# mehrnazmo/VIforSSMs

Hardware: AMD Instinct MI355X
Metric: latent-state transitions/sec (batch_dims×T per step), AR(1) T=5000, 1/2/4/8 GPU (higher is better)
Workload: dtype bf16

## Files before the change

viforssms_amd/csrc/flow_v5.hip:

```cpp
#include "flow5_api.hpp"

#ifndef VISSM_FLOW5_NS
#define VISSM_FLOW5_NS flow5
#define VISSM_FLOW5_BASE_UNIT 1
#endif

#include <cstdlib>
#ifndef VISSM_ABL_STORES
#define VISSM_ABL_STORES 0
#endif

namespace vissm {
namespace VISSM_FLOW5_NS {

constexpr int P = 16;
constexpr int HP = 64;
constexpr int S = 16;
constexpr int NW = 4;
constexpr int NT = 64 * NW;
constexpr int UW = 128;
constexpr int DTH = 56;

typedef __bf16 bf4 __attribute__((ext_vector_type(4)));
typedef __bf16 bf8 __attribute__((ext_vector_type(8)));
// ... 949 lines not shown
                for (int j = 0; j + w2 < KF; j += 2 * w2) t[j] += t[j + w2];
              v = t[0];
            } else {
#pragma unroll 4
              for (int j = 0; j < a.k; ++j) v += dsc[j * QW + qc];
            }
          } else {
#pragma unroll
            for (int p = 0; p < P; ++p) {
              const int j = q - a.s * p;
              const bool ok = static_cast<unsigned>(j) < static_cast<unsigned>(a.k);
              const float x = dsc[(ok ? j : 0) * QW + p];
              v += ok ? x : 0.f;
            }
          }
          const int oq2 = q - a.k;
          if (oq2 >= 0 && oq2 < fin) {
            if (a.s == 1) v += gw[oq2] * gsc[w][0][oq2];
            else v += (oq2 & 1) ? gw[oq2] * gsc[w][0][oq2 >> 1] : gsc[w][2][oq2 >> 1];
          }
          const float cin = mycarry[bl * KP + (q < a.k ? q : 0)];
          if (q < a.k) v += cin;
          if (q < fin) db[t0 + q] = v;
          else if (q < fin + a.k) mycarry[bl * KP + q - fin] = v;
        }
      }
    }
    if (c < nP) {
      const size_t row = (static_cast<size_t>(grp) * a.Lh + m0 + c) * a.H;
      if (a.dc16) {
        __bf16* dcs = reinterpret_cast<__bf16*>(dC_slab) + row;
#pragma unroll
        for (int rb = 0; rb < 4; ++rb)
#pragma unroll
          for (int r = 0; r < 4; ++r) {
            const int h = swz(16 * rb + 4 * g + r);
            if (h < a.H) dcs[h] = static_cast<__bf16>(dCa[rb][r] * kLog2e);
          }
      } else {
        float* dcs = dC_slab + row;
#pragma unroll
        for (int rb = 0; rb < 4; ++rb)
#pragma unroll
          for (int r = 0; r < 4; ++r) {
            const int h = swz(16 * rb + 4 * g + r);
            if (h < a.H) dcs[h] = dCa[rb][r] * kLog2e;
          }
      }
    }
  }

  if constexpr (FZ) {
    if (lane < nb) {
      float v = 0.f;
#pragma unroll
      for (int cc = 0; cc < P; ++cc) v += zls[w][lane][cc];
      fz.lsl[static_cast<size_t>(chn) * a.B + b_lo + lane] = v;
    }
  }
  for (int bl = 0; bl < nb; ++bl) {
    const int b = b_lo + bl;
    for (int q = lane; q < a.k * wdu; q += 64) {
      const float v = mycarry[bl * KP + q];
      if (chn == a.n_chunks - 1) du[static_cast<size_t>(b) * a.pL + a.Lout + q] = v;
      else halo[(static_cast<size_t>(b) * a.n_chunks + chn) * a.k + q] = v;
    }
    if (lane < a.H) dth_slab[(static_cast<size_t>(chn) * a.B + b) * a.H + lane] = dthl[w][bl][swz(lane)] * kLog2e;
  }

  const int H = a.H;
  const int nW = a.k * H + NH * H * H + 3 * NH * H + 2 * H + 2;
  float* ws = dW_slab + static_cast<size_t>(item) * nW;
#pragma unroll
  for (int jb = 0; jb < JB; ++jb)
#pragma unroll
    for (int hb = 0; hb < 4; ++hb)
#pragma unroll
      for (int r = 0; r < 4; ++r) {
        const int j = 16 * jb + 4 * g + r, h = swz(16 * hb + c);
        if (j < a.k && h < H) ws[j * H + h] = dWe[jb][hb][r] * kLog2e;
      }
  const int off_w = a.k * H, off_b = off_w + NH * H * H;
#pragma unroll
  for (int l = 0; l < NH; ++l)
#pragma unroll
    for (int ib = 0; ib < 4; ++ib)
#pragma unroll
      for (int ob = 0; ob < 4; ++ob)
#pragma unroll
        for (int r = 0; r < 4; ++r) {
          const int hi = swz(16 * ib + 4 * g + r), ho = swz(16 * ob + c);
          if (ho < H) {
            if (hi < H) ws[off_w + (l * H + hi) * H + ho] = dW[l][ib][ob][r];
            else if (hi == 63) ws[off_b + l * H + ho] = dW[l][ib][ob][r] * kLog2e;
          }
        }
  for (int i = lane; i < 2 * NH * H; i += 64) ws[off_b + NH * H + i] = 0.f;
  const int off_h = off_b + 3 * NH * H;
  const int oh = GI ? c - 5 : c;
  if (oh == 0 || oh == 1) {
#pragma unroll
    for (int hb = 0; hb < 4; ++hb)
#pragma unroll
      for (int r = 0; r < 4; ++r) {
        const int h = swz(16 * hb + 4 * g + r);
        if (h < H) ws[off_h + h * 2 + oh] = dWh[hb][r] * kLn2;
        else if (h == 63) ws[off_h + 2 * H + oh] = dWh[hb][r];
      }
  }
}

constexpr int NW2 = 8;
constexpr int NT2 = 64 * NW2;
__device__ __forceinline__ float swap_hi_lo(float v) {
  const auto r = __builtin_amdgcn_permlane32_swap(__builtin_bit_cast(unsigned, v), __builtin_bit_cast(unsigned, v),
                                                  false, false);
  return __builtin_bit_cast(float, static_cast<unsigned>(r[1]));
}
constexpr int KP2 = 8;
#ifndef VISSM_NODU_FENCES
#define VISSM_NODU_FENCES 1
#endif
template <bool FZ>
__device__ __forceinline__ void fence2() {
  if constexpr (FZ) fence();
}
#ifndef VISSM_BWD2_AHEAD
#define VISSM_BWD2_AHEAD 2
#endif
#ifndef VISSM_BWD2_AHEAD_VAR
#define VISSM_BWD2_AHEAD_VAR 6
#endif
#ifndef VISSM_BWD2_TAIL_DU
#define VISSM_BWD2_TAIL_DU 5
#endif
#ifndef VISSM_BWD2_TAIL_FZ
#define VISSM_BWD2_TAIL_FZ 59
#endif
#ifndef VISSM_BWD2_TAIL_NODU
#define VISSM_BWD2_TAIL_NODU 4
#endif
#ifndef VISSM_STAGE_AHEAD
#define VISSM_STAGE_AHEAD 1
#endif
#ifndef VISSM_STAGE_AHEAD_VAR
#define VISSM_STAGE_AHEAD_VAR 12
#endif
#ifndef VISSM_STAGE_SITE_DU
#define VISSM_STAGE_SITE_DU 0
#endif
#ifndef VISSM_STAGE_SITE_FZ
#define VISSM_STAGE_SITE_FZ 2
#endif
__device__ __forceinline__ unsigned lds_addr(const void* p) {
  return __builtin_amdgcn_readfirstlane(
      static_cast<unsigned>(reinterpret_cast<size_t>((__attribute__((address_space(3))) const void*)p)));
}
__device__ __forceinline__ void lds_dma_pair(unsigned long long mask0, unsigned long long mask1, unsigned voff,
                                             const float* base0, const float* base1, unsigned dst0, unsigned dst1) {
  unsigned keep_m0;
  unsigned long long keep_exec;
  asm volatile(
      "s_nop 4\n\t"
      "s_mov_b32 %0, m0\n\t"
      "s_and_saveexec_b64 %1, %2\n\t"
      "s_mov_b32 m0, %7\n\t"
      "s_nop 0\n\t"
      "global_load_lds_dword %4, %5\n\t"
      "s_and_b64 exec, %1, %3\n\t"
      "s_mov_b32 m0, %8\n\t"
      "s_nop 0\n\t"
      "global_load_lds_dword %4, %6\n\t"
      "s_mov_b64 exec, %1\n\t"
      "s_mov_b32 m0, %0"
      : "=&s"(keep_m0), "=&s"(keep_exec)
      : "s"(mask0), "s"(mask1), "v"(voff), "s"(base0), "s"(base1), "s"(dst0), "s"(dst1)
      : "memory", "scc");
}
__device__ __forceinline__ unsigned long long lanes_below(int n, bool on) {
  return on ? (n >= 64 ? ~0ull : (1ull << n) - 1ull) : 0ull;
}
template <int N>
__device__ __forceinline__ void stage_windows(const float* src, int pitch, int len, int b0, int b1, int t0, int n,
                                              int lane, float (*win)[N], bool on, bool both) {
  const unsigned long long m = lanes_below(n, on);
  lds_dma_pair(m, both ? m : 0ull, 4u * static_cast<unsigned>(clampi(t0 + lane, len)),
               src + static_cast<size_t>(b0) * pitch, src + static_cast<size_t>(b1) * pitch, lds_addr(win[0]),
               lds_addr(win[1]));
}
__device__ __forceinline__ void stage_wait() { asm volatile("s_waitcnt vmcnt(0)" ::: "memory"); }

constexpr int kSgMfma = 0x008, kSgDsRead = 0x100;
template <int ID, int N, int M>
__device__ __forceinline__ void sg_batch() {
  __builtin_amdgcn_sched_group_barrier(kSgDsRead, N, ID);
#pragma unroll
  for (int i = 0; i < N; ++i) __builtin_amdgcn_sched_group_barrier(kSgMfma, M, ID);
}
template <int ID, int NR, int NM>
__device__ __forceinline__ void sg_seq() {
  __builtin_amdgcn_sched_group_barrier(kSgDsRead, NR, ID);
  __builtin_amdgcn_sched_group_barrier(kSgMfma, NM, ID);
}

__device__ __forceinline__ bf8 cat8(bf4 a, bf4 b) {
  return __builtin_shufflevector(a, b, 0, 1, 2, 3, 4, 5, 6, 7);
}
__device__ __forceinline__ bf8 tr_frag2(const __bf16* img, int hb, int g, int c) {
  return cat8(tr_read(img, hb, g, c), tr_read(img + P * HP, hb, g, c));
}

#define VISSM_UW (*(STG ? &uwin[pw + w] : &uwin[w]))
#define VISSM_GW (*(STGG ? &gwin[pw + w] : &gwin[w]))
template <bool FZ, bool DU, bool TF, int NPR = 1, bool SB = false>
__global__ __launch_bounds__(NT2, 2) void bwd2_kernel(KArgs a, const float* __restrict__ u, const float* __restrict__ C,
                                                      const float* __restrict__ tht, const float* __restrict__ gout,
                                                      const float* __restrict__ dls, const bf8* __restrict__ img,
                                                      const float* __restrict__ cst, float* __restrict__ du,
                                                      float* __restrict__ dC_slab, float* __restrict__ dth_slab,
                                                      float* __restrict__ dW_slab, float* __restrict__ halo,
                                                      const u4* __restrict__ thf, FzArgs fz = FzArgs{}) {
  static_assert(!SB || NPR == 2, "the split backward chain goes with the split recompute");
  constexpr int NH = 1, KB = 1, JB = 1, NP = 1;
  constexpr bool LOF = NPR == 2 && !kLoFoldOff;
  constexpr bool AH =
      VISSM_BWD2_AHEAD && NPR == 1 && (FZ || TF) && (VISSM_BWD2_AHEAD_VAR & (FZ ? 4 : DU ? 2 : 1)) != 0;
  constexpr int TAIL = (VISSM_BWD2_AHEAD >= 2 && NPR == 1 && TF)
                           ? (FZ ? VISSM_BWD2_TAIL_FZ : DU ? VISSM_BWD2_TAIL_DU : VISSM_BWD2_TAIL_NODU) : 0;
  constexpr int PO = FZ ? P - 1 : P;
  constexpr int QW2 = P + KP2;
  constexpr int UWN = NPR == 2 ? 48 : 64;
  __shared__ Shared<NH, KB, JB, NP> sh;
  __shared__ __bf16 timg[NW2][2][2 * P * HP];
  __shared__ float dthl[NW2][S][DTH];
  __shared__ __attribute__((aligned(16))) float dths[NW2][4];
  __shared__ float carry[NW2][S][KP2];
  constexpr bool STG = VISSM_STAGE_AHEAD && NPR == 1 && TF && UWN == 64 &&
                       (VISSM_STAGE_AHEAD_VAR & (FZ ? 8 : DU ? 4 : 2)) != 0;
  constexpr bool STGG = STG && !FZ;
  constexpr int SITE = FZ ? VISSM_STAGE_SITE_FZ : VISSM_STAGE_SITE_DU;
  __shared__ float uwin[STG ? 2 * NW2 : NW2][2][UWN];
  __shared__ float gwin[STGG ? 2 * NW2 : NW2][2][P];
  __shared__ float gsc[NPR == 2 ? 1 : NW2][2][P];
  __shared__ float dscr[NW2][2][KP2][QW2];
  constexpr bool ZLS = FZ && NPR == 1;
  __shared__ float zls[ZLS ? NW2 : 1][ZLS ? S : 1][P];
  constexpr int RO = NPR == 2 ? 10 : 0, NLO = RO + (SB ? 10 : 0);
  __shared__ bf8 slo[NLO > 0 ? NLO : 1][64];
  __shared__ bf8 swe[NPR == 2 ? 4 : 1][16];
  __shared__ float zcar[FZ ? NW2 : 1][FZ ? S : 1];
  if constexpr (NPR == 2) {
    constexpr int NFR = Shared<NH, KB, JB, NP>::NFR;
    for (int i = threadIdx.x; i < NFR * 64; i += NT2) sh.img[i >> 6][0][i & 63] = img[((i >> 6) * 2) * 64 + (i & 63)];
    for (int i = threadIdx.x; i < NLO * 64; i += NT2) {
      const int j = i >> 6;
      const int f = j < 8 ? j
                  : j < 10 ? 16 * NH + 4 * KB + 2 * JB + (j - 8)
                  : j < 18 ? 8 * NH + (j - 10)
                           : 16 * NH + 4 * KB + (j - 18);
      slo[j][i & 63] = img[(f * 2 + 1) * 64 + (i & 63)];
    }
    for (int i = threadIdx.x; i < 4 * 16; i += NT2) swe[i >> 4][i & 15] = img[((16 * NH + (i >> 4)) * 2 + 1) * 64 + (i & 15)];
    for (int i = threadIdx.x; i < Shared<NH, KB, JB, NP>::NCST; i += NT2) sh.cst[i] = cst[i];
  } else {
    load_shared<NH, KB, JB, NP, NT2>(sh, img, cst);
  }
  if constexpr (FZ) {
    if constexpr (ZLS)
      for (int i = threadIdx.x; i < NW2 * S * P; i += NT2) (&zls[0][0][0])[i] = 0.f;
    for (int i = threadIdx.x; i < NW2 * S; i += NT2) (&zcar[0][0])[i] = 0.f;
  }
  for (int i = threadIdx.x; i < NW2 * S * DTH; i += NT2) (&dthl[0][0][0])[i] = 0.f;
  for (int i = threadIdx.x; i < NW2 * S * KP2; i += NT2) (&carry[0][0][0])[i] = 0.f;
  for (int i = threadIdx.x; i < NW2 * 2 * KP2 * QW2; i += NT2) (&dscr[0][0][0][0])[i] = 0.f;
  __syncthreads();
  const int w = threadIdx.x >> 6, lane = threadIdx.x & 63, c = lane & 15, g = lane >> 4;
  const int item = __builtin_amdgcn_readfirstlane(blockIdx.x * NW2 + w);
  const int grp = __builtin_amdgcn_readfirstlane(item / a.n_chunks);
  const int chn = __builtin_amdgcn_readfirstlane(item % a.n_chunks);
  if (grp >= a.n_groups) return;
  const int m_lo = chn * a.CH, m_hi = min(a.Lh, m_lo + a.CH);
  const int b_lo = grp * a.S, nb = min(a.S, a.B - b_lo);
  __bf16* const im0 = timg[w][0];
  __bf16* const im1 = timg[w][1];
  const unsigned* whp = reinterpret_cast<const unsigned*>(&sh.cst[NH * HP]);

  f4 dW[4][4], dWe[4], dWh[4];
#pragma unroll
  for (int i = 0; i < 4; ++i) {
#pragma unroll
    for (int o = 0; o < 4; ++o) dW[i][o] = f4{0.f, 0.f, 0.f, 0.f};
    dWe[i] = f4{0.f, 0.f, 0.f, 0.f};
    dWh[i] = f4{0.f, 0.f, 0.f, 0.f};
  }
  const int fwc = 16 * NH + 4 * KB;
  bf8 sel_p;
#pragma unroll
  for (int jj = 0; jj < 8; ++jj) sel_p[jj] = (__bf16)((4 * g + (jj & 3) == c) ? 1.f : 0.f);

  const float ldl = (!FZ && lane < nb) ? dls[b_lo + lane] : 0.f;
  float lt0 = 0.f, lt1 = 0.f, lis = 0.f;
  if constexpr (FZ) {
    if (lane < nb) {
      const float* tp = fz.theta + static_cast<size_t>(b_lo + lane) * 3;
      lt0 = tp[0];
      lt1 = tp[1];
      lis = __expf(-tp[2]);
    }
  }
  const int m_start = (FZ && chn > 0) ? m_lo - PO : m_lo;
  const int nu = a.k + P;
  int par = 0;
  if constexpr (STG) {
    if (lane >= nu) {
#pragma unroll
      for (int cb = 0; cb < 2; ++cb) {
        uwin[w][cb][lane] = 0.f;
        uwin[NW2 + w][cb][lane] = 0.f;
      }
    }
    stage_windows(u, a.pL, a.L, b_lo, b_lo + (1 < nb ? 1 : 0), m_start, nu, lane, uwin[w], m_start < m_hi, true);
    if constexpr (!FZ)
      stage_windows(gout, a.pLo, a.Lout, b_lo, b_lo + (1 < nb ? 1 : 0), m_start, P, lane, gwin[w], m_start < m_hi,
                    1 < nb);
  }
  for (int m0 = m_start; m0 < m_hi; m0 += PO) {
    const bool discard = FZ && m0 < m_lo;
    const int nP = discard ? 0 : min(PO, m_hi - m0), t0 = m0;
    const int nZ = FZ ? min(P, a.Lh - m0) : nP;
    f4 dCa[4];
#pragma unroll
    for (int rb = 0; rb < 4; ++rb) dCa[rb] = f4{0.f, 0.f, 0.f, 0.f};
    float fz_yt = 0.f, fz_bt = 0.f;
    if constexpr (FZ) {
      const int wo = min(max(m0 + c - 1, 0), fz.M - 1);
      fz_yt = fz.obs[wo];
      fz_bt = fz.bin[wo];
    }
    for (int bl = 0; bl < nb; bl += 2) {
      fence2<FZ || (!DU && VISSM_NODU_FENCES)>();
      const bool two = bl + 1 < nb;
      const int blv[2] = {bl, two ? bl + 1 : bl};
      const int bv[2] = {b_lo + blv[0], b_lo + blv[1]};
      int pw = 0;
      if constexpr (STG) {
        stage_wait();
        pw = par * NW2;
        asm volatile("" : "+s"(pw));
      }
      const auto stage_next = [&]() {
        const bool lastp = bl + 2 >= nb, more = !lastp || m0 + PO < m_hi;
        const int ms = (lastp && more) ? m0 + PO : m0, bs = lastp ? (more ? 0 : bl) : bl + 2;
        const int b0 = b_lo + bs, b1 = b_lo + (bs + 1 < nb ? bs + 1 : bs);
        __builtin_amdgcn_sched_barrier(0);
        stage_windows(u, a.pL, a.L, b0, b1, ms, nu, lane, uwin[NW2 - pw + w], more, true);
        if constexpr (STGG)
          stage_windows(gout, a.pLo, a.Lout, b0, b1, ms, P, lane, gwin[NW2 - pw + w], more, bs + 1 < nb);
        __builtin_amdgcn_sched_barrier(0);
      };
      (void)stage_next;
      f4 X[2][4];
      bf8 tfr[2];
      float fz_yp = fz_yt, fz_bp = fz_bt, fz_zc[2] = {0.f, 0.f};
      {
        float uv[2] = {0.f, 0.f}, gv[2] = {0.f, 0.f};
        if constexpr (!STG) {
#pragma unroll
          for (int cb = 0; cb < 2; ++cb) {
            const float* ub = u + static_cast<size_t>(bv[cb]) * a.pL;
            uv[cb] = lane < nu ? ub[clampi(t0 + lane, a.L)] : 0.f;
            if constexpr (!FZ) {
              if (lane < P) gv[cb] = gout[static_cast<size_t>(bv[cb]) * a.pLo + clampi(t0 + lane, a.Lout)];
            }
          }
          if (!two) gv[1] = 0.f;
        }
        const f4* crow = reinterpret_cast<const f4*>(C + static_cast<size_t>(m0 + clampi(c, nZ)) * HP) + g;
        f4 cr[4], tr[2][4];
        if constexpr (TF) {
#pragma unroll
          for (int cb = 0; cb < 2; ++cb) tfr[cb] = __builtin_bit_cast(bf8, thf[2 * static_cast<size_t>(bv[cb]) + (g & 1)]);
        }
#pragma unroll
        for (int rb = 0; rb < 4; ++rb) {
          cr[rb] = crow[4 * rb];
          if constexpr (!TF) {
#pragma unroll
            for (int cb = 0; cb < 2; ++cb)
              tr[cb][rb] = (reinterpret_cast<const f4*>(tht + static_cast<size_t>(bv[cb]) * HP) + g)[4 * rb];
          }
        }
        __builtin_amdgcn_sched_barrier(0);
        if constexpr (STG) {
          if constexpr (!FZ) {
            if (!two && lane < P) VISSM_GW[1][lane] = 0.f;
          } else {
            asm volatile("" : "+v"(fz_yp), "+v"(fz_bp));
          }
        }
#pragma unroll
        for (int cb = 0; cb < 2; ++cb) {
          if constexpr (!STG) {
            if (UWN == 64 || lane < UWN) VISSM_UW[cb][lane] = uv[cb];
            if (lane < P) VISSM_GW[cb][lane] = gv[cb];
          }
#pragma unroll
          for (int rb = 0; rb < 4; ++rb) X[cb][rb] = TF ? cr[rb] : cr[rb] + tr[cb][rb];
        }
        if constexpr (FZ) {
          fz_zc[0] = zcar[w][blv[0]];
          fz_zc[1] = zcar[w][blv[1]];
        }
      }
      u2 i0p[2][4];
      u2 d0p[2][4], d1p[2][4];
      float mu[2], rr[2];
      float uk_e = 0.f;
      {
        f4 acc[2][4];
        fence2<FZ || (!DU && VISSM_NODU_FENCES)>();
        const int gu = (LOF && g == 1) ? 0 : g;
        Fr8<NP> uf[2] = {u_frag<NP>(VISSM_UW[0], 1, 0, gu, c), u_frag<NP>(VISSM_UW[1], 1, 0, gu, c)};
        if constexpr (TF) {
          if (g >= 2) {
            uf[0].h = tfr[0];
            uf[1].h = tfr[1];
          }
        }
        if constexpr (AH) {
          bf8 we[4];
#pragma unroll
          for (int ob = 0; ob < 4; ++ob) we[ob] = sh.img[16 * NH + ob][0][lane];
          if constexpr ((TAIL & 8) != 0) __builtin_amdgcn_sched_barrier(0);
#pragma unroll
          for (int ob = 0; ob < 4; ++ob)
#pragma unroll
            for (int cb = 0; cb < 2; ++cb) acc[cb][ob] = mfma32(we[ob], uf[cb].h, X[cb][ob]);
          if constexpr ((TAIL & 8) == 0) sg_batch<1, 4, 2>();
        } else {
#pragma unroll
          for (int ob = 0; ob < 4; ++ob) {
            const Fr8<NP> wf = wfrag(sh, 16 * NH + ob, lane);
            bf8 wel = {};
            if constexpr (NPR == 2 && !LOF) {
              const bf8 v = swe[ob][c];
              if (g == 0) wel = v;
            }
#pragma unroll
            for (int cb = 0; cb < 2; ++cb) {
              acc[cb][ob] = X[cb][ob];
              if constexpr (NPR == 2 && !LOF) acc[cb][ob] = mfma32(wel, uf[cb].h, acc[cb][ob]);
              acc[cb][ob] = mm<NP>(wf, uf[cb], acc[cb][ob]);
            }
          }
        }
#pragma unroll
        for (int cb = 0; cb < 2; ++cb)
#pragma unroll
          for (int rb = 0; rb < 4; ++rb) {
            float e[4] = {0.f, 0.f, 0.f, 0.f};
#pragma unroll
            for (int r = 0; r < 4; ++r) {
              if (VISSM_DERIV16 >= 1) X[cb][rb][r] = 4 * rb + r < NR ? elu_dv(acc[cb][rb][r], e[r]) : 0.f;
              else X[cb][rb][r] = 4 * rb + r < NR ? elu_fast<true>(acc[cb][rb][r]) : 0.f;
            }
            if (VISSM_DERIV16 >= 1) {
              d0p[cb][rb] = u2{pk_f16(e[0], e[1]), 4 * rb + 2 < NR ? pk_f16(e[2], e[3]) : 0u};
              pin_pair(d0p[cb][rb]);
            }
          }
        fence2<FZ || (!DU && VISSM_NODU_FENCES)>();
        if constexpr (STG && SITE == 0) stage_next();
#pragma unroll
        for (int cb = 0; cb < 2; ++cb) {
          if (g == 3) X[cb][3][3] = 1.f;
#pragma unroll
          for (int ob = 0; ob < 4; ++ob) acc[cb][ob] = f4{0.f, 0.f, 0.f, 0.f};
        }
#pragma unroll
        for (int ks = 0; ks < 2; ++ks) {
          Fr8<NP> xf[2] = {chain_frag<NP>(X[0], ks), chain_frag<NP>(X[1], ks)};
          if constexpr (AH) {
            bf8 wq[4];
#pragma unroll
            for (int ob = 0; ob < 4; ++ob) wq[ob] = sh.img[ob * 2 + ks][0][lane];
#pragma unroll
            for (int ob = 0; ob < 4; ++ob)
#pragma unroll
              for (int cb = 0; cb < 2; ++cb) acc[cb][ob] = mfma32(wq[ob], xf[cb].h, acc[cb][ob]);
            if (ks == 0) sg_batch<2, 4, 2>();
            else sg_batch<3, 4, 2>();
          } else {
#pragma unroll
            for (int ob = 0; ob < 4; ++ob) {
              const Fr8<NP> wf = wfrag(sh, ob * 2 + ks, lane);
#pragma unroll
              for (int cb = 0; cb < 2; ++cb) {
                if constexpr (NPR == 2) acc[cb][ob] = mfma32(slo[ob * 2 + ks][lane], xf[cb].h, acc[cb][ob]);
                acc[cb][ob] = mm<NP>(wf, xf[cb], acc[cb][ob]);
              }
            }
          }
        }
#pragma unroll
        for (int cb = 0; cb < 2; ++cb) {
          put_image<NP>(im0 + cb * P * HP, nullptr, X[cb], g, c);
          if (VISSM_DERIV16 == 0) {
#pragma unroll
            for (int rb = 0; rb < 4; ++rb) i0p[cb][rb] = u2{cvt2(X[cb][rb][0], X[cb][rb][1]), cvt2(X[cb][rb][2], X[cb][rb][3])};
          }
        }
#pragma unroll
        for (int cb = 0; cb < 2; ++cb)
#pragma unroll
          for (int rb = 0; rb < 4; ++rb) {
            float e[4] = {0.f, 0.f, 0.f, 0.f};
#pragma unroll
            for (int r = 0; r < 4; ++r) {
              if (VISSM_DERIV16 >= 2) X[cb][rb][r] = 4 * rb + r < NR ? elu_dv(acc[cb][rb][r], e[r]) : 0.f;
              else X[cb][rb][r] = 4 * rb + r < NR ? elu_fast<true>(acc[cb][rb][r]) : 0.f;
            }
            if (VISSM_DERIV16 >= 2) {
              d1p[cb][rb] = u2{pk_f16(e[0], e[1]), 4 * rb + 2 < NR ? pk_f16(e[2], e[3]) : 0u};
              pin_pair(d1p[cb][rb]);
            }
          }
        fence2<FZ || (!DU && VISSM_NODU_FENCES)>();
        const int fh = 16 * NH + 4 * KB + 2 * JB;
        f4 d[2] = {f4{0.f, 0.f, 0.f, 0.f}, f4{0.f, 0.f, 0.f, 0.f}};
#pragma unroll
        for (int cb = 0; cb < 2; ++cb)
          if (g == 3) X[cb][3][3] = 1.f;
        if constexpr (FZ && (TAIL & 32) != 0) uk_e = VISSM_UW[g >> 1][c + a.k];
        if constexpr (AH) {
          const bf8 wh[2] = {sh.img[fh][0][lane], sh.img[fh + 1][0][lane]};
#pragma unroll
          for (int ks = 0; ks < 2; ++ks)
#pragma unroll
// ... 161 lines not shown
      for (int ks = 0; ks < 2; ++ks) {
        Fr8<NP> df[2] = {chain_frag<NP>(D[0], ks), chain_frag<NP>(D[1], ks)};
        if constexpr (AH) {
          bf8 wq[4];
#pragma unroll
          for (int ib = 0; ib < 4; ++ib) wq[ib] = sh.img[8 * NH + ib * 2 + ks][0][lane];
          if constexpr ((TAIL & 16) != 0) __builtin_amdgcn_sched_barrier(0);
#pragma unroll
          for (int ib = 0; ib < 4; ++ib)
#pragma unroll
            for (int cb = 0; cb < 2; ++cb) dX[cb][ib] = mfma32(wq[ib], df[cb].h, dX[cb][ib]);
          if constexpr ((TAIL & 16) != 0) {
          } else if (ks == 0) sg_batch<5, 4, 2>();
          else sg_batch<6, 4, 2>();
        } else {
#pragma unroll
          for (int ib = 0; ib < 4; ++ib) {
            const Fr8<NP> wb = wfrag(sh, 8 * NH + ib * 2 + ks, lane);
#pragma unroll
            for (int cb = 0; cb < 2; ++cb) {
              if constexpr (SB) dX[cb][ib] = mfma32(slo[RO + ib * 2 + ks][lane], df[cb].h, dX[cb][ib]);
              dX[cb][ib] = mm<NP>(wb, df[cb], dX[cb][ib]);
            }
          }
        }
      }
      fence2<FZ || (!DU && VISSM_NODU_FENCES)>();
      {
        bf8 dzf[4];
#pragma unroll
        for (int ob = 0; ob < 4; ++ob) dzf[ob] = tr_frag2(im1, ob, g, c);
        if constexpr (AH) {
          bf8 xa[4];
#pragma unroll
          for (int ib = 0; ib < 4; ++ib) xa[ib] = tr_frag2(im0, ib, g, c);
#pragma unroll
          for (int ib = 0; ib < 4; ++ib)
#pragma unroll
            for (int ob = 0; ob < 4; ++ob) dW[ib][ob] = mfma32(xa[ib], dzf[ob], dW[ib][ob]);
          sg_seq<9, 16, 16>();
        } else {
#pragma unroll
          for (int ib = 0; ib < 4; ++ib) {
            const bf8 xa = tr_frag2(im0, ib, g, c);
#pragma unroll
            for (int ob = 0; ob < 4; ++ob) dW[ib][ob] = mfma32(xa, dzf[ob], dW[ib][ob]);
          }
        }
      }
      bf8 uaf_e = {};
      if constexpr ((TAIL & 4) != 0) {
        const Fr4<NP> ua = ua_frag<NP>(VISSM_UW[0], 1, 0, g, c), ub = ua_frag<NP>(VISSM_UW[1], 1, 0, g, c);
        uaf_e = cat8(ua.h, ub.h);
      }
#pragma unroll
      for (int cb = 0; cb < 2; ++cb)
#pragma unroll
        for (int rb = 0; rb < 4; ++rb) {
          if (VISSM_DERIV16 >= 1) {
#pragma unroll
            for (int r = 0; r < 4; ++r) D[cb][rb][r] = 4 * rb + r < NR ? mul_h(dX[cb][rb][r], d0p[cb][rb][r >> 1], r & 1) : 0.f;
          } else {
            const f4 x = {__builtin_bit_cast(float, i0p[cb][rb][0] << 16), __builtin_bit_cast(float, i0p[cb][rb][0] & 0xffff0000u),
                          __builtin_bit_cast(float, i0p[cb][rb][1] << 16), __builtin_bit_cast(float, i0p[cb][rb][1] & 0xffff0000u)};
#pragma unroll
            for (int r = 0; r < 4; ++r) D[cb][rb][r] = 4 * rb + r < NR ? dX[cb][rb][r] * elu_d(x[r]) : 0.f;
          }
        }
      f4 dcn[2] = {f4{0.f, 0.f, 0.f, 0.f}, f4{0.f, 0.f, 0.f, 0.f}};
      if constexpr (DU && AH) {
        const bf8 wc[2] = {sh.img[fwc][0][lane], sh.img[fwc + 1][0][lane]};
#pragma unroll
        for (int ks = 0; ks < 2; ++ks)
#pragma unroll
          for (int cb = 0; cb < 2; ++cb) dcn[cb] = mfma32(wc[ks], chain_frag<NP>(D[cb], ks).h, dcn[cb]);
        sg_batch<7, 2, 2>();
      } else if constexpr (DU) {
#pragma unroll
        for (int ks = 0; ks < 2; ++ks) {
          const Fr8<NP> wc = wfrag(sh, fwc + ks, lane);
#pragma unroll
          for (int cb = 0; cb < 2; ++cb) {
            const Fr8<NP> dk = chain_frag<NP>(D[cb], ks);
            if constexpr (SB) dcn[cb] = mfma32(slo[RO + 8 + ks][lane], dk.h, dcn[cb]);
            dcn[cb] = mm<NP>(wc, dk, dcn[cb]);
          }
        }
      }
      if constexpr (FZ && !ZLS) {
#pragma unroll
        for (int cb = 0; cb < 2; ++cb) {
          const float hi = bf16_hi(lsv[cb]);
          D[cb][3][1] = g == 0 ? hi : (g == 1 ? lsv[cb] - hi : 0.f);
        }
      }
#pragma unroll
      for (int cb = 0; cb < 2; ++cb) put_image<NP>(im1 + cb * P * HP, nullptr, D[cb], g, c);
      if constexpr (DU) {
        if (g < KP2 / 4) {
#pragma unroll
          for (int cb = 0; cb < 2; ++cb)
#pragma unroll
            for (int r = 0; r < 4; ++r) dscr[w][cb][4 * g + r][c + 4 * g + r] = dcn[cb][r];
        }
      }
      float dut[KP2], dug = 0.f, dus = 0.f, duc = 0.f;
      const auto du_rows = [&]() {
        const int cbq = lane >> 5, q = lane & 31;
        const int qc = q < QW2 ? q : QW2 - 1;
#pragma unroll
        for (int j = 0; j < KP2; ++j) dut[j] = dscr[w][cbq][j][qc];
      };
      const auto du_terms = [&]() {
        const int cbq = lane >> 5, q = lane & 31;
        const int oqc = min(max(q - a.k, 0), P - 1);
        dug = VISSM_GW[cbq][oqc];
        dus = gsc[w][cbq][oqc];
        duc = carry[w][cbq ? blv[1] : blv[0]][q & (KP2 - 1)];
      };
      if constexpr (DU && (TAIL & 1) != 0) du_rows();
      if constexpr (DU && (TAIL & 2) != 0) du_terms();
      fence2<FZ || (!DU && VISSM_NODU_FENCES)>();
      {
        const unsigned one2 = 0x3F803F80u;
        bf8 uaf = uaf_e;
        if constexpr ((TAIL & 4) == 0) {
          const Fr4<NP> ua = ua_frag<NP>(VISSM_UW[0], 1, 0, g, c), ub = ua_frag<NP>(VISSM_UW[1], 1, 0, g, c);
          uaf = cat8(ua.h, ub.h);
        }
        bf8 bcomb = uaf;
        {
          const unsigned ta_ = c - 8 == (blv[0] & 7) ? one2 : 0u, tb_ = (two && c - 8 == (blv[1] & 7)) ? one2 : 0u;
          if (c >= 8) bcomb = __builtin_bit_cast(bf8, u4{ta_, ta_, tb_, tb_});
        }
        if constexpr (AH) {
          bf8 ta[4];
#pragma unroll
          for (int hb = 0; hb < 4; ++hb) ta[hb] = tr_frag2(im1, hb, g, c);
#pragma unroll
          for (int hb = 0; hb < 4; ++hb) {
            dWe[hb] = mfma32(ta[hb], bcomb, dWe[hb]);
            dCa[hb] = mfma32(ta[hb], sel_p, dCa[hb]);
          }
          sg_seq<10, 8, 8>();
        } else {
#pragma unroll
          for (int hb = 0; hb < 4; ++hb) {
            const bf8 ta = tr_frag2(im1, hb, g, c);
            dWe[hb] = mfma32(ta, bcomb, dWe[hb]);
            dCa[hb] = mfma32(ta, sel_p, dCa[hb]);
          }
        }
      }
      {
        if ((bl & 7) == 6 || bl + 2 >= nb) {
          const int smp = (bl & ~7) + c - 8;
          if (c >= 8 && smp < nb) {
            float* base = &dthl[w][smp][4 * g];
            f4* dp[4];
#pragma unroll
            for (int hb = 0; hb < 4; ++hb)
              dp[hb] = reinterpret_cast<f4*>(16 * hb + 4 * g < DTH ? base + 16 * hb : &dths[w][0]);
            f4 o[4];
#pragma unroll
            for (int hb = 0; hb < 4; ++hb) o[hb] = *dp[hb];
#pragma unroll
            for (int hb = 0; hb < 4; ++hb) *dp[hb] = o[hb] + dWe[hb];
          }
#pragma unroll
          for (int hb = 0; hb < 4; ++hb)
            if (c >= 8) dWe[hb] = f4{0.f, 0.f, 0.f, 0.f};
        }
      }
      if constexpr (DU) {
        fence2<FZ || (!DU && VISSM_NODU_FENCES)>();
        const int cbq = lane >> 5, q = lane & 31;
        const int lim = nP + a.k;
        const bool act = q < lim && (cbq == 0 || two);
        const int blq = cbq ? blv[1] : blv[0];
        float v = 0.f;
        if (act) {
          const int qc = q < QW2 ? q : QW2 - 1;
          float t[KP2];
#pragma unroll
          for (int j = 0; j < KP2; ++j) t[j] = (TAIL & 1) ? dut[j] : dscr[w][cbq][j][qc];
#pragma unroll
          for (int w2 = 1; w2 < KP2; w2 *= 2)
#pragma unroll
            for (int j = 0; j + w2 < KP2; j += 2 * w2) t[j] += t[j + w2];
          v = t[0];
          const int oq2 = q - a.k;
          if constexpr ((TAIL & 2) != 0) {
            if (oq2 >= 0 && oq2 < nP) v += dug * dus;
            if (q < a.k) v += duc;
          } else {
            if (oq2 >= 0 && oq2 < nP)
              v += NPR == 2 ? VISSM_GW[cbq][oq2] : VISSM_GW[cbq][oq2] * gsc[w][cbq][oq2];
            if (q < a.k) v += carry[w][blq][q];
          }
        }
        if (act) {
          float* const dur = du + static_cast<size_t>(b_lo + blq) * a.pL + t0;
          if (q < nP) {
            if constexpr (!(VISSM_ABL_STORES & 2)) dur[q] = v;
          } else {
            carry[w][blq][q - nP] = v;
          }
        }
      }
      if constexpr (STG) par ^= 1;
    }
    if (c < nP && !(VISSM_ABL_STORES & 4)) {
      const size_t row = (static_cast<size_t>(grp) * a.Lh + m0 + c) * a.H;
      if (a.dc16) {
        __bf16* dcs = reinterpret_cast<__bf16*>(dC_slab) + row;
#pragma unroll
        for (int rb = 0; rb < 4; ++rb)
#pragma unroll
          for (int r = 0; r < 4; ++r) {
            const int h = swz(16 * rb + 4 * g + r);
            if (h < a.H) dcs[h] = static_cast<__bf16>(dCa[rb][r] * kLog2e);
          }
      } else {
        float* dcs = dC_slab + row;
#pragma unroll
        for (int rb = 0; rb < 4; ++rb)
#pragma unroll
          for (int r = 0; r < 4; ++r) {
            const int h = swz(16 * rb + 4 * g + r);
            if (h < a.H) dcs[h] = dCa[rb][r] * kLog2e;
          }
      }
    }
  }

  if constexpr (FZ) {
    if (lane < nb) {
      float v = 0.f;
      if constexpr (!ZLS) {
        v = dthl[w][lane][49] + dthl[w][lane][53];
      } else {
#pragma unroll
        for (int cc = 0; cc < P; ++cc) v += zls[w][lane][cc];
      }
      fz.lsl[static_cast<size_t>(chn) * a.B + b_lo + lane] = v;
    }
  }
  for (int bl = 0; bl < nb; ++bl) {
    const int b = b_lo + bl;
    if constexpr (DU) {
      if (lane < a.k) {
        const float v = carry[w][bl][lane];
        if (chn == a.n_chunks - 1) du[static_cast<size_t>(b) * a.pL + a.Lout + lane] = v;
        else halo[(static_cast<size_t>(b) * a.n_chunks + chn) * a.k + lane] = v;
      }
    }
    if (lane < a.H) dth_slab[(static_cast<size_t>(chn) * a.B + b) * a.H + lane] = dthl[w][bl][swz(lane)] * kLog2e;
  }

  const int H = a.H;
  const int nW = a.k * H + NH * H * H + 3 * NH * H + 2 * H + 2;
  float* ws = dW_slab + static_cast<size_t>(item) * nW;
#pragma unroll
  for (int hb = 0; hb < 4; ++hb)
#pragma unroll
    for (int r = 0; r < 4; ++r) {
      const int ht = swz(16 * hb + 4 * g + r);
      if (c < a.k && ht < H) ws[c * H + ht] = dWe[hb][r] * kLog2e;
    }
  const int off_w = a.k * H, off_b = off_w + NH * H * H;
#pragma unroll
  for (int ib = 0; ib < 4; ++ib)
#pragma unroll
    for (int ob = 0; ob < 4; ++ob)
#pragma unroll
      for (int r = 0; r < 4; ++r) {
        const int hi = swz(16 * ib + 4 * g + r), ho = swz(16 * ob + c);
        if (ho < H) {
          if (hi < H) ws[off_w + hi * H + ho] = dW[ib][ob][r];
          else if (hi == 63) ws[off_b + ho] = dW[ib][ob][r] * kLog2e;
        }
      }
  for (int i = lane; i < 2 * NH * H; i += 64) ws[off_b + NH * H + i] = 0.f;
  const int off_h = off_b + 3 * NH * H;
  const int oh = c - 5;
  if (oh == 0 || oh == 1) {
#pragma unroll
    for (int hb = 0; hb < 4; ++hb)
#pragma unroll
      for (int r = 0; r < 4; ++r) {
        const int h = swz(16 * hb + 4 * g + r);
        if (h < H) ws[off_h + h * 2 + oh] = dWh[hb][r] * kLn2;
        else if (h == 63) ws[off_h + 2 * H + oh] = dWh[hb][r];
      }
  }
}

template <bool TF, int NP, int NH, int JB, int NWF = NW, bool LOF = false>
__global__ __launch_bounds__(64 * NWF, 2) void fwd2_kernel(KArgs a, const float* __restrict__ u,
                                                                  const float* __restrict__ C,
                                                                  const float* __restrict__ tht,
                                                                  const bf8* __restrict__ img,
                                                                  const float* __restrict__ cst,
                                                                  float* __restrict__ u_next,
                                                                  float* __restrict__ ls_slab,
                                                                  const u4* __restrict__ thf) {
  constexpr int KB = (JB + 1) / 2;
  __shared__ Shared<NH, KB, JB, NP> sh;
  constexpr bool STG = VISSM_STAGE_AHEAD && (VISSM_STAGE_AHEAD_VAR & 1) != 0 && TF && NP == 1 && NH == 1 && JB == 1 &&
                       NWF == NW && !LOF;
  __shared__ float uwin[STG ? 2 * NWF : NWF][2][64 * KB];
  load_shared<NH, KB, JB, NP, 64 * NWF>(sh, img, cst);
  {
    const int r = __builtin_amdgcn_readfirstlane(blockIdx.x / a.ncu) & 3;
    if (r == 1) __builtin_amdgcn_s_setprio(1);
    else if (r == 2) __builtin_amdgcn_s_setprio(2);
    else if (r == 3) __builtin_amdgcn_s_setprio(3);
  }
  __syncthreads();
  const int w = threadIdx.x >> 6, lane = threadIdx.x & 63, c = lane & 15, g = lane >> 4;
  const int item = __builtin_amdgcn_readfirstlane(blockIdx.x * NWF + w);
  if (item >= a.n_items) return;
  const int grp = item / a.n_chunks, ch = item % a.n_chunks;
  const int m_lo = ch * a.CH, m_hi = min(a.Lh, m_lo + a.CH);
  const int b_lo = grp * a.S, nb = min(a.S, a.B - b_lo);
  constexpr bool HIREG = NWF == NW;
  constexpr int NWR = HIREG ? 8 * NH + 4 * KB + 2 : 1;
  bf8 wr[NWR];
  constexpr bool HIDREG = !HIREG && LOF && VISSM_X2_HIDREG;
  bf8 wrh[HIDREG ? 8 * NH : 1];
  if constexpr (HIDREG) {
#pragma unroll
    for (int i = 0; i < 8 * NH; ++i) wrh[i] = sh.img[i][0][lane];
  }
  if constexpr (HIREG) {
#pragma unroll
    for (int i = 0; i < 8 * NH; ++i) wr[i] = sh.img[i][0][lane];
#pragma unroll
    for (int i = 0; i < 4 * KB; ++i) wr[8 * NH + i] = sh.img[16 * NH + i][0][lane];
#pragma unroll
    for (int i = 0; i < 2; ++i) wr[8 * NH + 4 * KB + i] = sh.img[16 * NH + 4 * KB + 2 * JB + i][0][lane];
  }
  auto W = [&](int f, int i) -> Fr8<NP> {
    Fr8<NP> r;
    if constexpr (HIREG) r.h = wr[i];
    else if (HIDREG && f < 8 * NH) r.h = wrh[HIDREG ? f : 0];
    else r.h = sh.img[f][0][lane];
    if constexpr (NP == 2) r.l = sh.img[f][1][lane];
    return r;
  };
  auto mmw = [](const Fr8<NP>& a, const bf8& b, f4 cc) -> f4 {
    if constexpr (NP == 2) cc = mfma32(a.l, b, cc);
    return mfma32(a.h, b, cc);
  };
  const int ss = NH == 1 ? 1 : a.s;
  const bool swp = NH == 1 ? false : a.swap_out != 0;
  const int nu = ss * P + a.k;
  int par = 0;
  if constexpr (STG) {
    if (lane >= nu) {
#pragma unroll
      for (int cb = 0; cb < 2; ++cb) {
// ... 1135 lines not shown
```

Baseline: 4.520 billion.

## Prefetch C rows ahead and cache theta fragments in LDS for DU backward

For the DU backward variant, theta fragments are loaded once per batch chunk into shared memory instead of being reloaded from global memory on every pair iteration. The C-row loads for the next iteration are also issued a step early into registers. The staging wait is relaxed to vmcnt(4) so these in-flight prefetches do not block the window DMA wait. This aims to hide global-load latency at the head of each iteration, at the cost of extra registers and a fragile dependence on the exact count of outstanding loads.

```diff
diff --git a/viforssms_amd/csrc/flow_v5.hip b/viforssms_amd/csrc/flow_v5.hip
--- a/viforssms_amd/csrc/flow_v5.hip
+++ b/viforssms_amd/csrc/flow_v5.hip
@@ -1125,6 +1125,27 @@
 #ifndef VISSM_STAGE_SITE_FZ
 #define VISSM_STAGE_SITE_FZ 2
 #endif
+#ifndef VISSM_HEAD_AHEAD
+#define VISSM_HEAD_AHEAD 1
+#endif
+#ifndef VISSM_HEAD_PIECES_NODU
+#define VISSM_HEAD_PIECES_NODU 0
+#endif
+#ifndef VISSM_HEAD_PIECES_DU
+#define VISSM_HEAD_PIECES_DU 3
+#endif
+#ifndef VISSM_HEAD_PIECES_FZ
+#define VISSM_HEAD_PIECES_FZ 0
+#endif
+#ifndef VISSM_HEAD_SITE_DU
+#define VISSM_HEAD_SITE_DU 1
+#endif
+#ifndef VISSM_HEAD_SITE_FZ
+#define VISSM_HEAD_SITE_FZ 0
+#endif
+#ifndef VISSM_HEAD_SITE_NODU
+#define VISSM_HEAD_SITE_NODU 0
+#endif
 __device__ __forceinline__ unsigned lds_addr(const void* p) {
   return __builtin_amdgcn_readfirstlane(
       static_cast<unsigned>(reinterpret_cast<size_t>((__attribute__((address_space(3))) const void*)p)));
@@ -1162,6 +1183,7 @@
                lds_addr(win[1]));
 }
 __device__ __forceinline__ void stage_wait() { asm volatile("s_waitcnt vmcnt(0)" ::: "memory"); }
+__device__ __forceinline__ void stage_wait_c4() { asm volatile("s_waitcnt vmcnt(4)" ::: "memory"); }
 
 constexpr int kSgMfma = 0x008, kSgDsRead = 0x100;
 template <int ID, int N, int M>
@@ -1215,6 +1237,12 @@
   __shared__ float uwin[STG ? 2 * NW2 : NW2][2][UWN];
   __shared__ float gwin[STGG ? 2 * NW2 : NW2][2][P];
   __shared__ float gsc[NPR == 2 ? 1 : NW2][2][P];
+  constexpr int HA = (VISSM_HEAD_AHEAD && NPR == 1 && TF)
+                         ? (FZ ? VISSM_HEAD_PIECES_FZ : DU ? VISSM_HEAD_PIECES_DU : VISSM_HEAD_PIECES_NODU) : 0;
+  constexpr bool THL = (HA & 1) != 0;
+  constexpr bool CRA = (HA & 2) != 0;
+  constexpr int CSITE = FZ ? VISSM_HEAD_SITE_FZ : DU ? VISSM_HEAD_SITE_DU : VISSM_HEAD_SITE_NODU;
+  __shared__ u4 thl[THL ? NW2 : 1][THL ? S : 1][2];
   __shared__ float dscr[NW2][2][KP2][QW2];
   constexpr bool ZLS = FZ && NPR == 1;
   __shared__ float zls[ZLS ? NW2 : 1][ZLS ? S : 1][P];
@@ -1284,6 +1312,9 @@
   const int m_start = (FZ && chn > 0) ? m_lo - PO : m_lo;
   const int nu = a.k + P;
   int par = 0;
+  if constexpr (THL) {
+    if (lane < 2 * nb) thl[w][lane >> 1][lane & 1] = thf[2 * static_cast<size_t>(b_lo) + lane];
+  }
   if constexpr (STG) {
     if (lane >= nu) {
 #pragma unroll
@@ -1296,6 +1327,17 @@
     if constexpr (!FZ)
       stage_windows(gout, a.pLo, a.Lout, b_lo, b_lo + (1 < nb ? 1 : 0), m_start, P, lane, gwin[w], m_start < m_hi,
                     1 < nb);
+  }
+  f4 crn[4] = {f4{0.f, 0.f, 0.f, 0.f}, f4{0.f, 0.f, 0.f, 0.f}, f4{0.f, 0.f, 0.f, 0.f}, f4{0.f, 0.f, 0.f, 0.f}};
+  const auto c_rows_next = [&](int mt) {
+    const int nZt = FZ ? min(P, a.Lh - mt) : min(PO, m_hi - mt);
+    const f4* cp = reinterpret_cast<const f4*>(C + static_cast<size_t>(mt + clampi(c, nZt)) * HP) + g;
+#pragma unroll
+    for (int rb = 0; rb < 4; ++rb) crn[rb] = cp[4 * rb];
+  };
+  (void)c_rows_next;
+  if constexpr (CRA) {
+    if (m_start < m_hi) c_rows_next(m_start);
   }
   for (int m0 = m_start; m0 < m_hi; m0 += PO) {
     const bool discard = FZ && m0 < m_lo;
@@ -1317,7 +1359,8 @@
       const int bv[2] = {b_lo + blv[0], b_lo + blv[1]};
       int pw = 0;
       if constexpr (STG) {
-        stage_wait();
+        if constexpr (CRA) stage_wait_c4();
+        else stage_wait();
         pw = par * NW2;
         asm volatile("" : "+s"(pw));
       }
@@ -1332,6 +1375,13 @@
         __builtin_amdgcn_sched_barrier(0);
       };
       (void)stage_next;
+      const auto c_rows_ahead = [&]() {
+        const bool lastp = bl + 2 >= nb;
+        __builtin_amdgcn_sched_barrier(0);
+        c_rows_next((lastp && m0 + PO < m_hi) ? m0 + PO : m0);
+        __builtin_amdgcn_sched_barrier(0);
+      };
+      (void)c_rows_ahead;
       f4 X[2][4];
       bf8 tfr[2];
       float fz_yp = fz_yt, fz_bp = fz_bt, fz_zc[2] = {0.f, 0.f};
@@ -1350,13 +1400,17 @@
         }
         const f4* crow = reinterpret_cast<const f4*>(C + static_cast<size_t>(m0 + clampi(c, nZ)) * HP) + g;
         f4 cr[4], tr[2][4];
-        if constexpr (TF) {
+        if constexpr (THL) {
+#pragma unroll
+          for (int cb = 0; cb < 2; ++cb) tfr[cb] = __builtin_bit_cast(bf8, thl[w][blv[cb]][g & 1]);
+        }
+        if constexpr (TF && !THL) {
 #pragma unroll
           for (int cb = 0; cb < 2; ++cb) tfr[cb] = __builtin_bit_cast(bf8, thf[2 * static_cast<size_t>(bv[cb]) + (g & 1)]);
         }
 #pragma unroll
         for (int rb = 0; rb < 4; ++rb) {
-          cr[rb] = crow[4 * rb];
+          cr[rb] = CRA ? crn[rb] : crow[4 * rb];
           if constexpr (!TF) {
 #pragma unroll
             for (int cb = 0; cb < 2; ++cb)
@@ -1824,6 +1878,7 @@
           }
         }
       }
+      if constexpr (CRA && CSITE == 2) c_rows_ahead();
       {
         if ((bl & 7) == 6 || bl + 2 >= nb) {
           const int smp = (bl & ~7) + c - 8;
@@ -1844,6 +1899,7 @@
             if (c >= 8) dWe[hb] = f4{0.f, 0.f, 0.f, 0.f};
         }
       }
+      if constexpr (CRA && CSITE == 1) c_rows_ahead();
       if constexpr (DU) {
         fence2<FZ || (!DU && VISSM_NODU_FENCES)>();
         const int cbq = lane >> 5, q = lane & 31;
@@ -1880,6 +1936,7 @@
           }
         }
       }
+      if constexpr (CRA && CSITE == 0) c_rows_ahead();
       if constexpr (STG) par ^= 1;
     }
     if (c < nP && !(VISSM_ABL_STORES & 4)) {
```

After: 4.538 billion, median of 6. No clear change (+0.4%).
